# dashpay/agora-blsful

Measured on AMD Instinct MI355X. Metric: BLS12-381 sig verifications/sec (batch), higher is better.
Workload: dtype u32

## Files before the change

### agora-blsful_amd/csrc/h2c.cuh

```cuda
#pragma once
#include "curve.cuh"
#include "tower_split.cuh"

struct sha256_ctx {
  uint32_t h[8];
  uint32_t w[16];
  uint32_t cur;
  uint32_t fill;
  uint32_t total;
};

BLS_CONST uint32_t SHA256_K[64] = {
    0x428a2f98, 0x71374491, 0xb5c0fbcf, 0xe9b5dba5, 0x3956c25b, 0x59f111f1, 0x923f82a4, 0xab1c5ed5, 0xd807aa98, 0x12835b01,
    0x243185be, 0x550c7dc3, 0x72be5d74, 0x80deb1fe, 0x9bdc06a7, 0xc19bf174, 0xe49b69c1, 0xefbe4786, 0x0fc19dc6, 0x240ca1cc,
    0x2de92c6f, 0x4a7484aa, 0x5cb0a9dc, 0x76f988da, 0x983e5152, 0xa831c66d, 0xb00327c8, 0xbf597fc7, 0xc6e00bf3, 0xd5a79147,
    0x06ca6351, 0x14292967, 0x27b70a85, 0x2e1b2138, 0x4d2c6dfc, 0x53380d13, 0x650a7354, 0x766a0abb, 0x81c2c92e, 0x92722c85,
    0xa2bfe8a1, 0xa81a664b, 0xc24b8b70, 0xc76c51a3, 0xd192e819, 0xd6990624, 0xf40e3585, 0x106aa070, 0x19a4c116, 0x1e376c08,
    0x2748774c, 0x34b0bcb5, 0x391c0cb3, 0x4ed8aa4a, 0x5b9cca4f, 0x682e6ff3, 0x748f82ee, 0x78a5636f, 0x84c87814, 0x8cc70208,
    0x90befffa, 0xa4506ceb, 0xbef9a3f7, 0xc67178f2};

BLS_FN uint32_t rotr32(uint32_t x, int n) { return (x >> n) | (x << (32 - n)); }

BLS_FN void sha256_rounds(uint32_t* h, const uint32_t* wsrc) {
  uint32_t w[16];
// ... 125 lines not shown
  uint32_t w[16];
  uint32_t nw;
};
BLS_FN void sha_words_block(sha_words& s) {
#if defined(__HIPCC__)
  u32x8_t hv;
  u32x16_t wv;
#pragma unroll
  for (int i = 0; i < 8; i++) hv[i] = s.h[i];
#pragma unroll
  for (int i = 0; i < 16; i++) wv[i] = s.w[i];
  hv = sha256_compress_v(hv, wv);
#pragma unroll
  for (int i = 0; i < 8; i++) s.h[i] = hv[i];
#else
  sha256_rounds(s.h, s.w);
#endif
}
BLS_FN void sha_words_init(sha_words& s) {
  s.h[0] = 0x6a09e667; s.h[1] = 0xbb67ae85; s.h[2] = 0x3c6ef372; s.h[3] = 0xa54ff53a;
  s.h[4] = 0x510e527f; s.h[5] = 0x9b05688c; s.h[6] = 0x1f83d9ab; s.h[7] = 0x5be0cd19;
#pragma unroll
  for (int i = 0; i < 16; i++) s.w[i] = 0;
  s.nw = 0;
}
BLS_FN void sha_words_feed(sha_words& s, uint32_t word) {
#pragma unroll
  for (int i = 0; i < 15; i++) s.w[i] = s.w[i + 1];
  s.w[15] = word;
  if (++s.nw == 16) {
    sha_words_block(s);
    s.nw = 0;
  }
}
BLS_FN uint32_t xmd_tail_word(uint32_t j, uint32_t nhead, uint32_t head, const uint8_t* dst, uint32_t dst_len) {
  uint32_t word = 0;
#pragma unroll
  for (int k = 0; k < 4; k++) {
    const uint32_t q = j + k;
    uint32_t b;
    if (q < nhead) b = (head >> (8 * (nhead - 1 - q))) & 0xffu;
    else if (q - nhead < dst_len) b = dst[q - nhead];
    else if (q - nhead == dst_len) b = dst_len;
    else if (q - nhead == dst_len + 1) b = 0x80u;
    else b = 0;
    word = (word << 8) | b;
  }
  return word;
}
BLS_FN void xmd_finish(sha_words& s, uint32_t before, uint32_t nhead, uint32_t head, const uint8_t* dst, uint32_t dst_len) {
  const uint32_t need = nhead + dst_len + 2, total = before + nhead + dst_len + 1;
  for (uint32_t j = 0; j < need || s.nw != 14; j += 4) sha_words_feed(s, xmd_tail_word(j, nhead, head, dst, dst_len));
  sha_words_feed(s, total >> 29);
  sha_words_feed(s, total << 3);
}
BLS_FN uint32_t be32_at(const uint8_t* p) { return ((uint32_t)p[0] << 24) | ((uint32_t)p[1] << 16) | ((uint32_t)p[2] << 8) | p[3]; }
template <int NOUT>
BLS_FN void expand_message_xmd_words(uint32_t* out, const uint8_t* pre, uint32_t pre_len, const uint8_t* m, uint32_t m_len,
                                     const uint8_t* dst, uint32_t dst_len) {
  if ((pre_len | m_len) & 3u) {
    uint8_t ub[NOUT];
    expand_message_xmd<NOUT>(ub, pre, pre_len, m, m_len, dst, dst_len);
    for (int i = 0; i < NOUT / 4; i++) out[i] = be32_at(ub + 4 * i);
    return;
  }
  sha_words s;
  sha_words_init(s);
  for (int i = 0; i < 16; i++) sha_words_feed(s, 0);
  for (uint32_t i = 0; i < pre_len; i += 4) sha_words_feed(s, be32_at(pre + i));
  if (((size_t)m & 3u) == 0) {
    for (uint32_t i = 0; i < m_len; i += 4) {
      const uint32_t v = *(const uint32_t*)(m + i);
      sha_words_feed(s, (v >> 24) | ((v >> 8) & 0xff00u) | ((v << 8) & 0xff0000u) | (v << 24));
    }
  } else {
    for (uint32_t i = 0; i < m_len; i += 4) sha_words_feed(s, be32_at(m + i));
  }
  xmd_finish(s, 64 + pre_len + m_len, 3, (uint32_t)NOUT << 8, dst, dst_len);
  uint32_t b0[8], bi[8];
#pragma unroll
  for (int i = 0; i < 8; i++) {
    b0[i] = s.h[i];
    bi[i] = 0;
  }
  const int TW = 24;
  const uint32_t need1 = dst_len + 3;
  const bool cached = need1 <= 4 * TW;
  uint32_t T[TW];
  if (cached) {
#pragma unroll
    for (int k = 0; k < TW; k++) T[k] = xmd_tail_word(4 * k, 1, 0, dst, dst_len);
  }
  for (int blk = 1; blk <= NOUT / 32; blk++) {
    sha_words_init(s);
#pragma unroll
    for (int i = 0; i < 8; i++) sha_words_feed(s, b0[i] ^ bi[i]);
    if (cached) {
#pragma unroll
      for (int k = 0; k < TW; k++)
        if (4u * k < need1 || s.nw != 14) sha_words_feed(s, k == 0 ? T[0] | ((uint32_t)blk << 24) : T[k]);
      while (s.nw != 14) sha_words_feed(s, 0);
      sha_words_feed(s, 0);
      sha_words_feed(s, (34 + dst_len) << 3);
    } else {
      xmd_finish(s, 32, 1, (uint32_t)blk, dst, dst_len);
    }
#pragma unroll
    for (int i = 0; i < 8; i++) {
      bi[i] = s.h[i];
      out[8 * (blk - 1) + i] = bi[i];
    }
  }
}
BLS_FN void fp_from_be64_words(fp& r, const uint32_t* wbe) {
  fp lo, hi, t, k;
  uint32_t w[12];
#pragma unroll
  for (int i = 0; i < 12; i++) w[i] = i < 4 ? wbe[3 - i] : 0;
  fp_set_words(hi, w);
#pragma unroll
  for (int i = 0; i < 12; i++) w[i] = wbe[15 - i];
  fp_set_words(lo, w);
  fp_load(k, FP_R2);
  fp_mul(t, k, lo);
  fp_load(k, FP_R2_384);
  fp_mul(hi, k, hi);
  fp_add(t, t, hi);
  fp_reduce(r, t);
}

BLS_FN void fp_from_be64(fp& r, const uint8_t* b) {
  fp lo, hi, t, k;
  uint32_t w[12];
  for (int i = 0; i < 12; i++) w[i] = 0;
  for (int i = 0; i < 4; i++) {
    const uint8_t* q = b + 4 * (3 - i);
    w[i] = ((uint32_t)q[0] << 24) | ((uint32_t)q[1] << 16) | ((uint32_t)q[2] << 8) | q[3];
  }
  fp_set_words(hi, w);
  for (int i = 0; i < 12; i++) {
    const uint8_t* q = b + 16 + 4 * (11 - i);
    w[i] = ((uint32_t)q[0] << 24) | ((uint32_t)q[1] << 16) | ((uint32_t)q[2] << 8) | q[3];
  }
  fp_set_words(lo, w);
  fp_load(k, FP_R2);
  fp_mul(t, k, lo);
  fp_load(k, FP_R2_384);
  fp_mul(hi, k, hi);
  fp_add(t, t, hi);
  fp_reduce(r, t);
}

template <class F>
BLS_NOINLINE void sswu_g1(F& xn, F& xd, F& y, const F& u) {
  F A, B, Z, tv1, tv2, tv3, tv4, tv5, tv6, x, y1, t;
  fp_load(A, SSWU1_A);
  fp_load(B, SSWU1_B);
  fp_load(Z, SSWU1_Z);
  fp_sqr(tv1, u);
  fp_mul(tv1, Z, tv1);
  fp_sqr(tv2, tv1);
  fp_add(tv2, tv2, tv1);
  fp_one(t);
  fp_add(tv3, tv2, t);
  fp_mul(tv3, B, tv3);
  fp_neg(tv4, tv2);
  fp_cmov(tv4, Z, fp_is_zero(tv2));
  fp_mul(tv4, A, tv4);
  fp_sqr(tv2, tv3);
  fp_sqr(tv6, tv4);
  fp_mul(tv5, A, tv6);
  fp_add(tv2, tv2, tv5);
  fp_mul(tv2, tv2, tv3);
  fp_mul(tv6, tv6, tv4);
  fp_mul(tv5, B, tv6);
  fp_add(tv2, tv2, tv5);
  fp_mul(x, tv1, tv3);
  F s1, s2, s3, y2, c2;
  fp_sqr(s1, tv6);
  fp_mul(s2, tv2, tv6);
  fp_mul(s1, s1, s2);
  fp_pow(y1, s1, EXP_PM3D4, EXP_PM3D4_BITS);
  fp_mul(y1, y1, s2);
  fp_load(c2, SSWU1_C2);
  fp_mul(y2, y1, c2);
  fp_sqr(s3, y1);
  fp_mul(s3, s3, tv6);
  bool is_qr = fp_eq(s3, tv2);
  fp_mul(y, tv1, u);
  fp_mul(y, y, y2);
  fp_cmov(x, tv3, is_qr);
  fp_cmov(y, y1, is_qr);
  F ny;
  fp_neg(ny, y);
  fp_cmov(y, ny, fp_parity(u) != fp_parity(y));
  xn = x;
  xd = tv4;
}

BLS_NOINLINE void iso_map_g1(g1_jac& r, const fp& xn, const fp& xd, const fp& y) {
  fp XN, XD, YN, YD, pw, c, t;
  fp_load(XN, ISO1_XNUM[11]);
  fp_load(XD, ISO1_XDEN[10]);
  fp_load(YN, ISO1_YNUM[15]);
  fp_load(YD, ISO1_YDEN[15]);
  pw = xd;
#pragma unroll
  for (int j = 1; j <= 15; j++) {
    if (j > 1) fp_mul(pw, pw, xd);
    if (j <= 11) {
      fp_mul(XN, XN, xn);
      fp_load(c, ISO1_XNUM[11 - j]);
      fp_mul(t, c, pw);
      fp_add(XN, XN, t);
    }
    if (j <= 10) {
      fp_mul(XD, XD, xn);
      fp_load(c, ISO1_XDEN[10 - j]);
      fp_mul(t, c, pw);
      fp_add(XD, XD, t);
    }
    fp_mul(YN, YN, xn);
    fp_load(c, ISO1_YNUM[15 - j]);
    fp_mul(t, c, pw);
    fp_add(YN, YN, t);
    fp_mul(YD, YD, xn);
    fp_load(c, ISO1_YDEN[15 - j]);
    fp_mul(t, c, pw);
    fp_add(YD, YD, t);
  }
  fp zx, yd2;
  fp_mul(zx, XD, xd);
  fp_mul(r.z, zx, YD);
  fp_sqr(yd2, YD);
  fp_mul(t, XN, zx);
  fp_mul(r.x, t, yd2);
  fp_sqr(t, zx);
  fp_mul(t, t, zx);
  fp_mul(t, t, yd2);
  fp_mul(t, t, YN);
  fp_mul(r.y, t, y);
}

#if defined(__HIPCC__)
__device__ __forceinline__ void fp_lane_swap(fp& r, const fp& a) {
#pragma unroll
  for (int i = 0; i < FP_NL; i++) r.l[i] = dpp_swap(a.l[i]);
}
__device__ __forceinline__ void jac_dbl_pair(g1_jac& p, bool hi) {
  fp s1, s2, s3, in, a, b, o2, o3, D, E, t, x3, y3, z3, c8;
  fp_sel(in, hi, p.y, p.x);
  fp_sqr(s1, in);
  fp_dbl(E, s1);
  fp_add(E, E, s1);
  fp_reduce(E, E);
  fp_sel(in, hi, s1, E);
  fp_sqr(s2, in);
  fp_add(t, p.x, s1);
  fp_sel(a, hi, t, p.y);
  fp_sel(b, hi, t, p.z);
  fp_mul(s3, a, b);
  fp_lane_swap(o2, s2);
  fp_lane_swap(o3, s3);
  fp_sub(t, o3, s1);
  fp_sub(t, t, o2);
  fp_dbl(D, t);
  fp_reduce(D, D);
  fp_dbl(t, D);
  fp_sub(t, s2, t);
  fp_reduce(x3, t);
  fp_sub(t, D, x3);
  fp_mul(t, E, t);
  fp_dbl(c8, o2);
  fp_dbl(c8, c8);
  fp_reduce(c8, c8);
  fp_dbl(c8, c8);
  fp_sub(t, t, c8);
  fp_reduce(y3, t);
  fp_dbl(z3, s3);
  fp_reduce(z3, z3);
  fp_lane_swap(a, x3);
  fp_lane_swap(b, y3);
  fp_lane_swap(t, z3);
  fp_sel(p.x, hi, a, x3);
  fp_sel(p.y, hi, b, y3);
  fp_sel(p.z, hi, t, z3);
}
__device__ __noinline__ void jac_mul_u64_pair(g1_jac& r, const g1_jac& p, uint64_t k, bool hi) {
  g1_jac acc;
  jac_set_inf(acc);
  for (int i = 63; i >= 0; i--) {
    jac_dbl_pair(acc, hi);
    if ((k >> i) & 1) jac_add_body(acc, acc, p);
  }
  r = acc;
}
#endif
BLS_NOINLINE void hash_to_g1(g1_jac& r, const uint8_t* pre, uint32_t pre_len, const uint8_t* m, uint32_t m_len,
                       const uint8_t* dst, uint32_t dst_len, int lane2 = -1, bool no_clear = false) {
  uint32_t ub[32];
  expand_message_xmd_words<128>(ub, pre, pre_len, m, m_len, dst, dst_len);
  fp u0, u1, xn, xd, y;
  g1_jac q0, q1;
#if defined(__HIPCC__)
  if (lane2 >= 0) {
    g1_jac mine, other;
    fp_from_be64_words(u0, ub + 16 * lane2);
    sswu_g1(xn, xd, y, u0);
    iso_map_g1(mine, xn, xd, y);
    fp_lane_swap(other.x, mine.x);
    fp_lane_swap(other.y, mine.y);
    fp_lane_swap(other.z, mine.z);
    q0 = lane2 ? other : mine;
    q1 = lane2 ? mine : other;
  } else
#endif
  {
    (void)lane2;
    fp_from_be64_words(u0, ub);
    fp_from_be64_words(u1, ub + 16);
    sswu_g1(xn, xd, y, u0);
    iso_map_g1(q0, xn, xd, y);
    sswu_g1(xn, xd, y, u1);
    iso_map_g1(q1, xn, xd, y);
  }
  jac_add(q0, q0, q1);
  if (no_clear) {
    r = q0;
    return;
  }
#if defined(__HIPCC__)
  if (lane2 >= 0) jac_mul_u64_pair(q1, q0, BLS_X_ABS, lane2 != 0);
  else
#endif
    jac_mul_u64(q1, q0, BLS_X_ABS);
  jac_add(r, q1, q0);
}

template <class F2>
BLS_NOINLINE void sswu_g2(F2& x, F2& y, const F2& u) {
  typedef decltype(F2::c0) F;
  F2 A, B, Z, tv1, tv2, xn, xd, xd2, xd3, num, w, t, Y;
  fp2_load(A, SSWU2_A);
  fp2_load(B, SSWU2_B);
  fp2_load(Z, SSWU2_Z);
  fp2_sqr(tv1, u);
  fp2_mul(tv1, Z, tv1);
  fp2_sqr(tv2, tv1);
  fp2_add(tv2, tv2, tv1);
  fp2_reduce(tv2, tv2);
  fp2_one(t);
  fp2_add(t, tv2, t);
  fp2_mul(xn, B, t);
  fp2_neg(t, tv2);
  fp2_cmov(t, Z, fp2_is_zero(tv2));
  fp2_mul(xd, A, t);
  fp2_sqr(xd2, xd);
  fp2_mul(xd3, xd2, xd);
  fp2_sqr(num, xn);
  fp2_mul(t, A, xd2);
  fp2_add(num, num, t);
  fp2_mul(num, num, xn);
  fp2_mul(t, B, xd3);
  fp2_add(num, num, t);
  fp2_mul(w, num, xd);
  F nxd, nt, inxd;
  fp_sqr(nxd, xd.c0);
  fp_sqr(nt, xd.c1);
  fp_add(nxd, nxd, nt);
  fp_reduce(nxd, nxd);
  F n, sn, c2, nu, nu3, cz, root;
  fp_sqr(n, w.c0);
  fp_sqr(nt, w.c1);
  fp_add(n, n, nt);
  fp_reduce(n, n);
  fp_pow(sn, n, EXP_PM3D4, EXP_PM3D4_BITS);
  fp_mul(sn, sn, n);
  fp_sqr(c2, sn);
  const bool sq1 = fp_eq(c2, n);
  fp_sqr(nu, u.c0);
  fp_sqr(nt, u.c1);
  fp_add(nu, nu, nt);
  fp_reduce(nu, nu);
  fp_sqr(nu3, nu);
  fp_mul(nu3, nu3, nu);
  fp_load(cz, SSWU2_CZ);
  fp_mul(root, sn, cz);
  fp_mul(root, root, nu3);
  fp_cmov(root, sn, sq1);
  {
    F2 t3, w2, xn2;
    fp2_sqr(t3, tv1);
    fp2_mul(t3, t3, tv1);
    fp2_mul(w2, w, t3);
    fp2_mul(xn2, tv1, xn);
    fp2_cmov(w2, w, sq1);
    fp2_cmov(xn2, xn, sq1);
    w = w2;
    xn = xn2;
  }
  if (fp_is_zero(w.c1)) {
    fp2_sqrt_inv(Y, w, &nxd, &inxd);
  } else {
    F h, tt, s, d, prod, pi;
    fp_load(h, FP_HALF);
    fp_add(tt, w.c0, root);
    fp_mul(tt, tt, h);
    fp_pow(s, tt, EXP_PM3D4, EXP_PM3D4_BITS);
    fp_mul(s, s, tt);
    fp_sqr(c2, s);
    const bool direct = fp_eq(c2, tt);
    fp_dbl(d, s);
    fp_reduce(d, d);
    fp_mul(prod, d, nxd);
    fp_inv(pi, prod);
    fp_mul(inxd, pi, d);
    fp_mul(d, pi, nxd);
    fp_mul(d, w.c1, d);
    Y.c0 = s;
    Y.c1 = d;
    F2 alt;
    alt.c0 = d;
    alt.c1 = s;
    fp2_cmov(Y, alt, !direct);
  }
  F2 xdi;
  fp2_conj(xdi, xd);
  fp2_mul_fp(xdi, xdi, inxd);
  fp2_mul(x, xn, xdi);
  fp2_sqr(t, xdi);
  fp2_mul(y, Y, t);
  if (fp2_sgn0(u) != fp2_sgn0(y)) fp2_neg(y, y);
}
template <class F2>
BLS_FN void iso2_poly(F2& r, const uint32_t (*k)[2 * FP_NL], int deg, const F2& x) {
  F2 acc, c;
  fp2_load(acc, k[deg]);
  for (int i = deg - 1; i >= 0; i--) {
    fp2_mul(acc, acc, x);
    fp2_load(c, k[i]);
    fp2_add(acc, acc, c);
  }
  r = acc;
}
BLS_NOINLINE void iso_map_g2(g2_jac& r, const fp2& x, const fp2& y) {
  fp2 XN, XD, YN, YD, t, yd2;
  iso2_poly(XN, ISO2_XNUM, 3, x);
  iso2_poly(XD, ISO2_XDEN, 2, x);
  iso2_poly(YN, ISO2_YNUM, 3, x);
  iso2_poly(YD, ISO2_YDEN, 3, x);
  fp2_mul(r.z, XD, YD);
  fp2_sqr(yd2, YD);
  fp2_mul(t, XN, XD);
  fp2_mul(r.x, t, yd2);
  fp2_sqr(t, XD);
  fp2_mul(t, t, XD);
  fp2_mul(t, t, yd2);
  fp2_mul(t, t, YN);
  fp2_mul(r.y, t, y);
}
template <class F2>
BLS_FN void iso_map_g2_hom(F2& X, F2& Y, F2& Z, const F2& x, const F2& y) {
  F2 XN, XD, YN, YD, t;
  iso2_poly(XN, ISO2_XNUM, 3, x);
  iso2_poly(XD, ISO2_XDEN, 2, x);
  iso2_poly(YN, ISO2_YNUM, 3, x);
  iso2_poly(YD, ISO2_YDEN, 3, x);
  fp2_mul(X, XN, YD);
  fp2_mul(t, YN, XD);
  fp2_mul(Y, t, y);
  fp2_mul(Z, XD, YD);
}
BLS_NOINLINE void hash_to_g2(g2_jac& r, const uint8_t* pre, uint32_t pre_len, const uint8_t* m, uint32_t m_len,
                       const uint8_t* dst, uint32_t dst_len, int lane2 = -1, bool no_clear = false) {
  uint32_t ub[64];
  expand_message_xmd_words<256>(ub, pre, pre_len, m, m_len, dst, dst_len);
  fp2 u0, u1, x, y;
  g2_jac q0, q1;
#if defined(__HIPCC__)
  if (lane2 >= 0) {
    g2_jac mine, other;
    fp_from_be64_words(u0.c0, ub + 32 * lane2);
    fp_from_be64_words(u0.c1, ub + 32 * lane2 + 16);
    sswu_g2(x, y, u0);
    iso_map_g2(mine, x, y);
    fp_lane_swap(other.x.c0, mine.x.c0);
    fp_lane_swap(other.x.c1, mine.x.c1);
    fp_lane_swap(other.y.c0, mine.y.c0);
    fp_lane_swap(other.y.c1, mine.y.c1);
    fp_lane_swap(other.z.c0, mine.z.c0);
// ... 40 lines not shown
```

### agora-blsful_amd/csrc/kernels.cuh

```cuda
#pragma once
#ifndef BLS_SPLIT_WAVES
#define BLS_SPLIT_WAVES 2
#endif
#include "verify.cuh"

#define BLS_BLOCK 64
#define W1 FP_NL
#define W2 (2 * FP_NL)
#define WS_PAIRS_WORDS (6 * W2)
#define WS_PAIR1_WORDS (3 * W2)
#define WS_F_WORDS (6 * W2)
#define LINE5_WORDS (5 * FP_NL)
#define LINE3_WORDS_H (3 * FP_NL)
#define FX_STORE_WORDS (10 * 6 * FP_NL)
#define MILLER1_GROUP 3

struct dst_arg {
  uint8_t b[256];
  uint32_t len;
};

__device__ __forceinline__ void ws_ld_fp(fp& r, const uint32_t* ws, size_t stride, size_t i, int w0) {
#pragma unroll
  for (int k = 0; k < FP_NL; k++) r.l[k] = (int32_t)ws[(size_t)(w0 + k) * stride + i];
// ... 196 lines not shown
}

template <int SG>
__global__ void k_prepare(size_t n, const uint8_t* pks, const uint8_t* sigs, int fmt, int aug, const uint8_t* msgs,
                          const uint64_t* offs, int single_msg, dst_arg dst, uint32_t* pairs, int32_t* status, int pre_status, int two_lanes);
__global__ void k_miller2s(size_t n, const uint32_t* pairs, const int32_t* status, uint32_t* fws, int fixed_g2);
__global__ void k_lines2s(size_t n, size_t first, size_t count, const uint32_t* pairs, const int32_t* status, uint32_t* lines, uint32_t* lines3, size_t lanes, int fixed_g2, int pass);
__global__ void k_millerf2s(size_t n, size_t first, size_t count, const int32_t* status, const uint32_t* lines, size_t lanes, uint32_t* fws);
__global__ void k_finalexp2s(size_t n, size_t first, size_t count, const uint32_t* fws, uint32_t* vp, size_t lanes, int32_t* status);
__global__ void k_finalexp_seg(int seg, size_t n, size_t first, size_t count, const uint32_t* fws, uint32_t* vp, size_t lanes, int32_t* status);
__global__ void k_cyc_run4(size_t count, uint32_t* vp, size_t lanes, const int32_t* status, size_t first);
__global__ void k_linesp(size_t mm, size_t half, size_t stride, const uint32_t* pairs, const int32_t* bad, uint32_t* lines, uint32_t* lines3, size_t lanes, size_t first_v, size_t count_v, int pass);
__global__ void k_linesp4(size_t cnt, size_t stride, const uint32_t* pairs, const int32_t* bad, uint32_t* lines3, size_t lanes);
__global__ void k_lines_fixed(size_t stride, const uint32_t* pairs, const int32_t* bad, uint32_t* lines3, size_t lanes, int fixed_g2);
__global__ void k_millerfp(size_t count_v, size_t q, int group, const uint32_t* lines, size_t lanes, uint32_t* fws, size_t stride, size_t out0);
__global__ void k_millerfp3(size_t count, size_t q, int group, const int32_t* bad, const uint32_t* lines3, size_t lanes, uint32_t* fws, size_t stride, size_t out0);
__global__ void k_line_quad(size_t count, size_t q, const int32_t* bad, const uint32_t* lines3, size_t lanes, uint32_t* fout, size_t sout, size_t rout, size_t oout);
__global__ void k_f12_fold4(size_t qin, size_t qout, int fan, const uint32_t* fin, size_t sin, size_t rin, uint32_t* fout, size_t sout, size_t rout, size_t oout);
__global__ void k_finalexps(size_t n, const uint32_t* fws, int32_t* status);
__global__ void k_miller1s(size_t n, size_t stride, const uint32_t* pairs, const int32_t* skip, uint32_t* fws);
__global__ void k_finalexp_ones(const uint32_t* fws, size_t stride, int32_t* verdict);
__global__ void k_pairing_coop(size_t n, const uint32_t* pairs, int32_t* status, int fixed_g2);
__global__ void k_finalexp_coop(const uint32_t* fws, size_t stride, int32_t* verdict);
template <int SG>
__global__ void k_prepare_agg(size_t n, const uint8_t* pks, const uint8_t* sig, int fmt, int aug, const uint8_t* msgs,
                              const uint64_t* offs, dst_arg dst, uint32_t* pairs, int32_t* bad, int two_lanes, int has_sig);
__global__ void k_pairs_to_affine(size_t n, const uint8_t* g1s, const uint8_t* g2s, int fmt, uint32_t* pairs, int32_t* skip);
__global__ void k_pairs2_to_affine(size_t n, const uint8_t* g1a, const uint8_t* g2a, const uint8_t* g1b, const uint8_t* g2b, int fmt,
                                   uint32_t* pairs, int32_t* status);
__global__ void k_status_to_flag(size_t n, int32_t* status);
template <int SG>
__global__ void k_prepare_hashed(size_t n, const uint8_t* pks, const uint8_t* sigs, const uint8_t* hashes, uint32_t* pairs, int32_t* status, int fmt);
template <int SG>
__global__ void k_prepare_proof(size_t n, const uint8_t* commitments, const uint8_t* proofs, const uint8_t* pks, const uint8_t* ys,
                                int fmt, const uint8_t* msgs, const uint64_t* offs, dst_arg dst, uint32_t* pairs, int32_t* status);
__global__ void k_f12_fold(size_t m, size_t half, uint32_t* fws, size_t stride);
#define GROUPED_ITEMS 8
template <int SG>
__global__ void k_prepare_grouped(size_t n, const uint8_t* pks, const uint8_t* sigs, int fmt, int aug, const uint8_t* msgs, const uint64_t* offs,
                                  dst_arg dst, uint64_t seed, size_t ng, uint32_t* pairs, int32_t* skip, uint8_t* scaled_sigs, int32_t* status);
__global__ void k_group_sigsum(size_t ng, size_t n, const uint8_t* scaled_sigs, uint32_t* pairs, int32_t* skip);
__global__ void k_f12_mul3(size_t ng, const uint32_t* fin, size_t stride_in, uint32_t* fout);
__global__ void k_f12_import(size_t n, const uint8_t* src, uint32_t* fws, size_t stride);
__global__ void k_f12_export(const uint32_t* fws, size_t stride, uint8_t* dst);
__global__ void k_hash_to_g1(size_t n, const uint8_t* msgs, const uint64_t* offs, dst_arg dst, uint8_t* out, int two_lanes);
__global__ void k_hash_to_g2(size_t n, const uint8_t* msgs, const uint64_t* offs, dst_arg dst, uint8_t* out, int two_lanes);
template <int G, int WITH_SCALARS>
__global__ void k_accumulate(size_t n, const uint8_t* pts, int fmt, const uint8_t* scalars, const uint32_t* perm,
                             uint8_t* partials, size_t T);
__global__ void k_accumulate_g2s(size_t n, const uint8_t* pts, int fmt, uint8_t* partials, size_t T);
template <int G>
__global__ void k_point_fold(size_t m, size_t half, uint8_t* partials);
__global__ void k_point_fold_g2s(size_t m, size_t half, uint8_t* partials);
template <int G>
__global__ void k_compress(size_t n, const uint8_t* pts, int fmt, int legacy, uint8_t* out);
template <int SG>
__global__ void k_sign(size_t n, const uint8_t* sks, int aug, const uint8_t* msgs, const uint64_t* offs, dst_arg dst,
                       uint8_t* out_pks, uint8_t* out_sigs);
__global__ void k_msm_count(size_t n, const uint8_t* scalars, int c, int W, int clast, uint32_t* cnt);
__global__ void k_msm_fill(size_t n, const uint8_t* scalars, int c, int W, int clast, const uint32_t* off, uint32_t* cursor, uint32_t* idx);
template <int G>
__global__ void k_msm_bucket(size_t nb, const uint8_t* pts, int fmt, const uint32_t* perm, const uint32_t* cnt, const uint32_t* off,
                             const uint32_t* idx, uint8_t* sums);
template <int G>
__global__ void k_msm_chunk(int c, int W, int clast, int CH, const uint8_t* sums, uint8_t* partials);
__global__ void k_msm_chunk_g2s(int c, int W, int clast, int CH, const uint8_t* sums, uint8_t* partials);
__global__ void k_msm_chunk_g1p(int c, int W, int clast, int CH, const uint8_t* sums, uint8_t* partials);
__global__ void k_msm_chunk_g2q(int c, int W, int clast, int CH, const uint8_t* sums, uint8_t* partials);
__global__ void k_msm_bucket_g2s(size_t nb, const uint8_t* pts, int fmt, const uint32_t* perm, const uint32_t* cnt, const uint32_t* off,
                                 const uint32_t* idx, uint8_t* sums);
template <int G>
__global__ void k_normalize(uint8_t* pt);
#define MSM2_E(G) ((G) == 1 ? 2 : 4)
#define MSM2_AFF_WORDS(G) ((G) == 1 ? 2 * FP_NL : 4 * FP_NL)
template <int G>
__global__ void k_msm2_prep(size_t n, const uint8_t* pts, int fmt, const uint32_t* perm, uint32_t* affws, uint8_t* inf);
template <int G>
__global__ void k_msm2_tables(size_t n, const uint32_t* affws, const uint8_t* inf, int W, uint32_t* tab, uint32_t* jt);
template <int G>
__global__ void k_msm2_count(size_t n, const uint8_t* scalars, const uint8_t* inf, int W, uint32_t* cnt, uint64_t* subs);
template <int G>
__global__ void k_msm2_fill(size_t n, const uint64_t* subs, const uint8_t* inf, int W, const uint32_t* off, uint32_t* cursor, uint32_t* idx);
__global__ void k_msm2_merge_g1(size_t nb, int Q, uint8_t* sums);
__global__ void k_msm2_merge_g2s(size_t nb, int Q, uint8_t* sums);
__global__ void k_msm2_bucket_g1(size_t nb, int Q, const uint32_t* affws, const uint32_t* cnt, const uint32_t* off, const uint32_t* idx, uint8_t* sums, int tabW);
__global__ void k_msm2_bucket_g2s(size_t nb, int Q, const uint32_t* affws, const uint32_t* cnt, const uint32_t* off, const uint32_t* idx, uint8_t* sums, int tabW);
__global__ void k_msm2_chunk_g1p(int W, int CH, int stride, const uint8_t* sums, uint8_t* partials, int weighted);
__global__ void k_msm2_chunk_g2q(int W, int CH, int stride, const uint8_t* sums, uint8_t* partials, int weighted);
template <int G>
__global__ void k_decompress(size_t n, const uint8_t* bytes, int legacy, uint8_t* out, int32_t* status, int keep);

#include "util_kernels.cuh"
__global__ void k_wide_mul_test(size_t n, const uint8_t* a, const uint8_t* b, uint8_t* out, int reps);
#include "wide_rows.cuh"
#define WIDE_BLOCK 256
#define WIDE_ENGINE_BLOCK (16 * WIDE_TABLE_ROWS)
#define WIDE_EASY_WORDS (12 * 16)
__global__ void k_pairing_coop_easy(size_t n, const uint32_t* pairs, const int32_t* status, int fixed_g2, uint32_t* easy);
__global__ void k_finalexp_wide(size_t n, const uint32_t* easy, int32_t* status);
__global__ void k_finalexp_wide_ws(const uint32_t* fws, size_t stride, int32_t* verdict);
__global__ void k_f12_tree_wide(size_t m, const uint32_t* fin, size_t sin, uint32_t* fout, size_t sout);
__global__ void k_f12_tree_seg(size_t qin, const uint32_t* fin, size_t sin, size_t rin, uint32_t* fout, size_t sout, size_t rout);
__global__ void k_f12_horner_wide(const uint32_t* fin, size_t sin, uint32_t* fout, size_t sout);
__global__ void k_wide_prog_test(const uint32_t* prog, int len, int reps, const uint8_t* fin, uint8_t* tout);
bool wide_prog_is_fp12(const uint32_t* prog, size_t len);
__global__ void k_pairing_wide(size_t n, const uint32_t* pairs, int32_t* status, int fixed_g2);
__global__ void k_hash_to_g1_wide(size_t n, const uint8_t* msgs, const uint64_t* offs, int single_msg, dst_arg dst, uint8_t* out, uint32_t* rec);
__global__ void k_hash_to_g1_engine(size_t n, const uint8_t* msgs, const uint64_t* offs, int single_msg, dst_arg dst, uint8_t* out, uint32_t* rec);
#define WREC_P0 0
#define WREC_P1 3
#define WREC_Q0 6
#define WREC_F1 12
#define WREC_L 24
#define WREC_Q1 (24 + 6 * 68)
#define WREC_F2 (WREC_Q1 + 6)
#define WREC_F2_SLOTS 2
#define WREC_VALUES (WREC_F2 + 12 * WREC_F2_SLOTS)
#define WREC_WORDS (16 * WREC_VALUES)
template <int SG>
__global__ void k_prepare_keys(size_t n, const uint8_t* pks, const uint8_t* sigs, const uint8_t* hashes, int fmt, int parts, uint32_t* rec, int32_t* status);
__global__ void k_pairing_pre(size_t n, uint32_t* rec, const int32_t* status, int first_part, int second_part);
__global__ void k_pairing_post(size_t n, const uint32_t* rec, int32_t* status);
#define WSTREAM_FLAGS 32
#define WSTREAM_MAX_ITEMS 64
#define WPOST2_MAX_ITEMS 128
#define WSTREAM_SPIN_LIMIT (1u << 21)
#define BLS_ERR_STREAM_TIMEOUT (-2)
__global__ void k_pairing_stream(size_t n, uint32_t* rec, int32_t* status, uint32_t* flags, uint32_t epoch);
__global__ void k_pairing_post2(size_t n, uint32_t* rec, int32_t* status, uint32_t* flags, uint32_t epoch);
template <int G>
__global__ void k_point_tree_wide(size_t m, const uint8_t* in, uint8_t* out);
__global__ void k_g2_clear_wide(size_t n, uint8_t* pts);
__global__ void k_hash_to_g2_engine(size_t n, const uint8_t* msgs, const uint64_t* offs, int single_msg, dst_arg dst, uint8_t* out, uint32_t* rec);
__global__ void k_hash_to_g2_maps(size_t n, const uint8_t* msgs, const uint64_t* offs, int single_msg, dst_arg dst, uint32_t* pts);
__global__ void k_g2_hash_tail_wide(size_t n, const uint32_t* pts, uint8_t* out, uint32_t* rec);

#if defined(BLS_TU_PREPARE1) || defined(BLS_TU_PREPARE2)
template <int SG>
__global__ void __launch_bounds__(BLS_BLOCK, 2) k_prepare(size_t n, const uint8_t* pks, const uint8_t* sigs, int fmt, int aug,
                                                     const uint8_t* msgs, const uint64_t* offs, int single_msg, dst_arg dst,
                                                     uint32_t* pairs, int32_t* status, int pre_status, int two_lanes) {
  const size_t gid = (size_t)blockIdx.x * blockDim.x + threadIdx.x;
  const bool tl = SG == 2 || (two_lanes & 1) != 0;
  const size_t i = tl ? gid >> 1 : gid;
  const int lane2 = tl ? (int)(gid & 1) : -1;
  if (i >= n) return;
  if (pre_status && status[i] != BLS_OK) return;
  size_t mi = single_msg ? 0 : i;
  const uint8_t* m = msgs + offs[mi];
  uint32_t mlen = (uint32_t)(offs[mi + 1] - offs[mi]);
  g1_aff P[2];
  g2_aff Q[2];
  int st;
  if (SG == 1 && !aug) {
    fp zs;
    fp2 zp;
    load_g1_z(zs, sigs, i, fmt);
    load_g2_z(zp, pks, i, fmt);
    if (fp_is_zero(zs)) {
      st = BLS_ERR_SIG_IDENTITY;
    } else if (fp2_is_zero(zp)) {
      st = BLS_ERR_PK_IDENTITY;
    } else {
      const bool no_clear = (two_lanes & 2) != 0;
      g1_jac h;
      hash_to_g1(h, nullptr, 0, m, mlen, dst.b, dst.len, lane2, no_clear);
      g2_jac pk;
      g1_jac sig;
      load_g2_pt(pk, pks, i, fmt);
      load_g1_pt(sig, sigs, i, fmt);
      prepare_g1impl_tail(P, Q, pk, sig, h);
      if (no_clear) g2_negc_gen(Q[1]);
      else g2_neg_gen(Q[1]);
      st = BLS_OK;
    }
  } else if (SG == 1) {
    g2_jac pk;
    g1_jac sig;
    load_g2_pt(pk, pks, i, fmt);
    load_g1_pt(sig, sigs, i, fmt);
    st = prepare_g1impl(P, Q, pk, sig, aug, m, mlen, dst.b, dst.len, lane2, (two_lanes & 2) != 0);
  } else {
    g1_jac pk;
    g2_jac sig;
    load_g1_pt(pk, pks, i, fmt);
    load_g2_pt(sig, sigs, i, fmt);
    st = prepare_g2impl(P, Q, pk, sig, aug, m, mlen, dst.b, dst.len, lane2);
  }
  if (lane2 > 0) return;
  status[i] = st;
  if (st != BLS_OK) return;
  ws_st_pair(pairs, n, i, 0, P[0], Q[0]);
  ws_st_pair(pairs, n, i, 1, P[1], Q[1]);
}
__device__ __forceinline__ void sha256_u64(sha256_ctx& c, uint64_t x) {
  for (int k = 7; k >= 0; k--) sha256_byte(c, (uint8_t)(x >> (8 * k)));
}
struct u128_pair { uint64_t hi, lo; };
__device__ __noinline__ u128_pair grouped_scalar(uint64_t seed, size_t n, size_t i, const uint8_t* pk, uint32_t pk_len, const uint8_t* sig, uint32_t sig_len,
                                              const uint8_t* m, uint32_t mlen) {
  static_assert(GROUPED_ITEMS == 8 && BLS_BLOCK % GROUPED_ITEMS == 0, "a group is an aligned octet of lanes");
  uint8_t d[32];
  sha256_ctx c;
  if (i < n) {
    const char tag[] = "blsgpu-grouped-v3";
    sha256_init(c);
    sha256_update(c, (const uint8_t*)tag, sizeof tag - 1);
    sha256_u64(c, seed);
    sha256_u64(c, (uint64_t)n);
    sha256_u64(c, (uint64_t)i);
    sha256_update(c, pk, pk_len);
    sha256_update(c, sig, sig_len);
    sha256_u64(c, mlen);
    sha256_update(c, m, mlen);
    sha256_final(c, d);
  } else {
    for (int k = 0; k < 32; k++) d[k] = 0;
  }
  uint32_t w[8];
  for (int k = 0; k < 8; k++) w[k] = ((uint32_t)d[4 * k] << 24) | ((uint32_t)d[4 * k + 1] << 16) | ((uint32_t)d[4 * k + 2] << 8) | d[4 * k + 3];
  sha256_init(c);
  for (int j = 0; j < GROUPED_ITEMS; j++)
    for (int k = 0; k < 8; k++) {
      const uint32_t x = (uint32_t)__shfl((int)w[k], j, GROUPED_ITEMS);
      sha256_byte(c, (uint8_t)(x >> 24));
      sha256_byte(c, (uint8_t)(x >> 16));
      sha256_byte(c, (uint8_t)(x >> 8));
      sha256_byte(c, (uint8_t)x);
    }
  sha256_final(c, d);
  sha256_init(c);
  sha256_update(c, d, 32);
  sha256_u64(c, (uint64_t)i);
  sha256_final(c, d);
  u128_pair r{0, 0};
  for (int k = 0; k < 8; k++) r.hi = (r.hi << 8) | d[k];
  for (int k = 8; k < 16; k++) r.lo = (r.lo << 8) | d[k];
  if (!(r.hi | r.lo)) r.lo = 1;
  return r;
}
template <int SG>
__global__ void __launch_bounds__(BLS_BLOCK, 2) k_prepare_grouped(size_t n, const uint8_t* pks, const uint8_t* sigs, int fmt, int aug, const uint8_t* msgs,
                                                             const uint64_t* offs, dst_arg dst, uint64_t seed, size_t ng, uint32_t* pairs, int32_t* skip,
                                                             uint8_t* scaled_sigs, int32_t* status) {
  static_assert(SG == 1, "grouped verification is built for Bls12381G1Impl");
  const size_t i = (size_t)blockIdx.x * blockDim.x + threadIdx.x;
  const bool live = i < n;
  const size_t ii = live ? i : 0;
  const uint8_t* m = msgs + offs[ii];
  const uint32_t mlen = (uint32_t)(offs[ii + 1] - offs[ii]);
  const uint32_t pk_len = fmt == 0 ? 288 : 192, sig_len = fmt == 0 ? 144 : 96;
  const u128_pair r = grouped_scalar(seed, n, i, pks + ii * pk_len, pk_len, sigs + ii * sig_len, sig_len, m, mlen);
  if (!live) return;
  const size_t slot = i / GROUPED_ITEMS + (i % GROUPED_ITEMS) * ng, stride = (GROUPED_ITEMS + 1) * ng;
  g1_aff P[2];
  g2_aff Q[2];
  g2_jac pk;
  g1_jac sig, a, b;
  load_g2_pt(pk, pks, i, fmt);
  load_g1_pt(sig, sigs, i, fmt);
  const int st = prepare_g1impl(P, Q, pk, sig, aug, m, mlen, dst.b, dst.len, -1, true);
  status[i] = st;
  if (st != BLS_OK) {
    jac_set_inf(b);
    store_g1_pt(scaled_sigs, i, b);
    return;
  }
  jac_from_aff(a, P[0]);
  jac_mul_u128(a, a, r.hi, r.lo);
  jac_from_aff(b, P[1]);
  jac_mul_u128(b, b, r.hi, r.lo);
  g1_aff A;
  jac_to_aff(A, a);
  ws_st_pair(pairs, stride, slot, 0, A, Q[0]);
  skip[slot] = A.inf ? 1 : 0;
  store_g1_pt(scaled_sigs, i, b);
}
#if defined(BLS_TU_PREPARE1)
template __global__ void k_prepare_grouped<1>(size_t, const uint8_t*, const uint8_t*, int, int, const uint8_t*, const uint64_t*, dst_arg, uint64_t, size_t,
                                              uint32_t*, int32_t*, uint8_t*, int32_t*);
#endif
#if defined(BLS_TU_PREPARE1)
template __global__ void k_prepare<1>(size_t, const uint8_t*, const uint8_t*, int, int, const uint8_t*, const uint64_t*, int, dst_arg, uint32_t*, int32_t*, int, int);
#else
template __global__ void k_prepare<2>(size_t, const uint8_t*, const uint8_t*, int, int, const uint8_t*, const uint64_t*, int, dst_arg, uint32_t*, int32_t*, int, int);
#endif
#endif



#if defined(BLS_TU_AGG1) || defined(BLS_TU_AGG2) || defined(BLS_TU_AGG_BATCH)
template <int SG>
__device__ __forceinline__ void prepare_agg_item(bool is_sig, const uint8_t* pts, size_t pt_i, int fmt, int aug, const uint8_t* m, uint32_t mlen,
                                                 const dst_arg& dst, uint32_t* pairs, size_t stride, size_t slot, int32_t* bad, int two_lanes, int lane2) {
  g1_aff P;
  g2_aff Q;
  if (is_sig) {
    if (SG == 1) {
      g1_jac s;
      load_g1_pt(s, pts, pt_i, fmt);
      const bool inf = jac_is_inf(s);
      if (lane2 <= 0) bad[slot] = inf ? 1 : 0;
      if (inf) return;
      jac_to_aff(P, s);
      if (two_lanes & 2) g2_negc_gen(Q);
      else g2_neg_gen(Q);
    } else {
      g2_jac s;
      load_g2_pt(s, pts, pt_i, fmt);
      const bool inf = jac_is_inf(s);
      if (lane2 <= 0) bad[slot] = inf ? 1 : 0;
      if (inf) return;
      jac_to_aff(Q, s);
      g1_neg_gen(P);
    }
    if (lane2 <= 0) ws_st_pair(pairs, stride, slot, 0, P, Q);
    return;
  }
  if (SG == 1) {
    g2_jac pk;
    load_g2_pt(pk, pts, pt_i, fmt);
    const bool inf = jac_is_inf(pk);
    if (lane2 <= 0) bad[slot] = inf ? 1 : 0;
    if (inf) return;
    uint8_t pre[96];
    g1_jac h;
    if (aug) {
      jac_to_aff(Q, pk);
      g2_compress(pre, Q, false);
      hash_to_g1(h, pre, 96, m, mlen, dst.b, dst.len, lane2, (two_lanes & 2) != 0);
      jac_to_aff(P, h);
    } else {
      hash_to_g1(h, pre, 0, m, mlen, dst.b, dst.len, lane2, (two_lanes & 2) != 0);
      if (jac_is_inf(h)) {
// ... 3329 lines not shown
```

### agora-blsful_amd/csrc/verify.cuh

```cuda
#pragma once
#include "h2c.cuh"
#include "pairing.cuh"

#define BLS_OK 0
#define BLS_ERR_INVALID_SIGNATURE 1
#define BLS_ERR_SIG_IDENTITY 2
#define BLS_ERR_PK_IDENTITY 3
#define BLS_ERR_DUPLICATE_MESSAGE 4
#define BLS_ERR_INVALID_COEFFICIENT 5
#define BLS_ERR_BAD_LENGTH 6
#define BLS_ERR_BAD_ENCODING 7
#define BLS_ERR_LEGACY_FORMAT 8
#define BLS_ERR_COMMITMENT_IDENTITY 9
#define BLS_ERR_PROOF_IDENTITY 10
#define BLS_ERR_ZERO_CHALLENGE 11

BLS_FN void fp_inv3(fp& a, fp& b, fp& c) {
  fp ab, abc, t;
  fp_mul(ab, a, b);
  fp_mul(abc, ab, c);
  fp_inv(abc, abc);
  fp_mul(t, abc, ab);
  fp_mul(abc, abc, c);
  c = t;
  fp_mul(t, abc, b);
  fp_mul(b, abc, a);
  a = t;
}
BLS_FN void fp_inv2(fp& a, fp& b) {
  fp ab, t;
  fp_mul(ab, a, b);
  fp_inv(ab, ab);
  fp_mul(t, ab, b);
  fp_mul(b, ab, a);
  a = t;
}
BLS_FN void g1_apply_zinv(g1_aff& r, const g1_jac& p, const fp& zi) {
  fp zi2;
  fp_sqr(zi2, zi);
  fp_mul(r.x, p.x, zi2);
  fp_mul(zi2, zi2, zi);
  fp_mul(r.y, p.y, zi2);
  r.inf = false;
}
BLS_FN void g2_apply_ninv(g2_aff& r, const g2_jac& p, const fp& ni) {
  fp2 zi, zi2;
  fp_mul(zi.c0, p.z.c0, ni);
  fp_mul(zi.c1, p.z.c1, ni);
  fp_neg(zi.c1, zi.c1);
  fp2_sqr(zi2, zi);
  fp2_mul(r.x, p.x, zi2);
  fp2_mul(zi2, zi2, zi);
  fp2_mul(r.y, p.y, zi2);
  r.inf = false;
}
BLS_FN void fp2_norm_sq(fp& n, const fp2& a) {
  fp t;
  fp_sqr(n, a.c0);
  fp_sqr(t, a.c1);
  fp_add(n, n, t);
}

BLS_FN void g1g2_to_aff(g1_aff& a1, g2_aff& a2, const g1_jac& p1, const g2_jac& p2) {
  fp z1 = p1.z, n2;
  fp2_norm_sq(n2, p2.z);
  fp_inv2(z1, n2);
  g1_apply_zinv(a1, p1, z1);
  g2_apply_ninv(a2, p2, n2);
}

BLS_FN void g1_neg_gen(g1_aff& r) {
  fp_load(r.x, G1_GEN_X);
  fp y;
  fp_load(y, G1_GEN_Y);
  fp_neg(r.y, y);
  r.inf = false;
}
BLS_FN void g2_negc_gen(g2_aff& r) {
  fp2_load(r.x, G2_NEGC_X);
  fp2_load(r.y, G2_NEGC_Y);
  r.inf = false;
}
BLS_FN void g2_neg_gen(g2_aff& r) {
  fp2_load(r.x, G2_GEN_X);
  fp2 y;
  fp2_load(y, G2_GEN_Y);
  fp2_neg(r.y, y);
  r.inf = false;
}

BLS_FN void prepare_g1impl_tail(g1_aff* P, g2_aff* Q, const g2_jac& pk, const g1_jac& sig, const g1_jac& h) {
  if (jac_is_inf(h)) {
    g1g2_to_aff(P[1], Q[0], sig, pk);
    jac_to_aff(P[0], h);
  } else {
    fp zs = sig.z, zh = h.z, n;
    fp2_norm_sq(n, pk.z);
    fp_inv3(zs, zh, n);
    g1_apply_zinv(P[1], sig, zs);
    g1_apply_zinv(P[0], h, zh);
    g2_apply_ninv(Q[0], pk, n);
  }
}
BLS_FN int prepare_g1impl(g1_aff* P, g2_aff* Q, const g2_jac& pk, const g1_jac& sig, int mode, const uint8_t* msg,
                          uint32_t msg_len, const uint8_t* dst, uint32_t dst_len, int lane2 = -1, bool no_clear = false) {
  if (jac_is_inf(sig)) return BLS_ERR_SIG_IDENTITY;
  if (jac_is_inf(pk)) return BLS_ERR_PK_IDENTITY;
  g1_jac h;
  if (mode) {
    g1g2_to_aff(P[1], Q[0], sig, pk);
    uint8_t pre[96];
    g2_compress(pre, Q[0], false);
    if (mode == 1) hash_to_g1(h, pre, 96, msg, msg_len, dst, dst_len, lane2, no_clear);
    else hash_to_g1(h, nullptr, 0, pre, 96, dst, dst_len, lane2, no_clear);
    jac_to_aff(P[0], h);
  } else {
    hash_to_g1(h, nullptr, 0, msg, msg_len, dst, dst_len, lane2, no_clear);
    prepare_g1impl_tail(P, Q, pk, sig, h);
  }
  if (no_clear) g2_negc_gen(Q[1]);
  else g2_neg_gen(Q[1]);
  return BLS_OK;
}

BLS_FN int prepare_g2impl(g1_aff* P, g2_aff* Q, const g1_jac& pk, const g2_jac& sig, int mode, const uint8_t* msg,
                          uint32_t msg_len, const uint8_t* dst, uint32_t dst_len, int lane2 = -1) {
  if (jac_is_inf(sig)) return BLS_ERR_SIG_IDENTITY;
  if (jac_is_inf(pk)) return BLS_ERR_PK_IDENTITY;
  g2_jac h;
  if (mode) {
    g1g2_to_aff(P[0], Q[1], pk, sig);
    uint8_t pre[48];
    g1_compress(pre, P[0], false);
    if (mode == 1) hash_to_g2(h, pre, 48, msg, msg_len, dst, dst_len, lane2);
    else hash_to_g2(h, nullptr, 0, pre, 48, dst, dst_len, lane2);
    jac_to_aff(Q[0], h);
  } else {
    hash_to_g2(h, nullptr, 0, msg, msg_len, dst, dst_len, lane2);
    if (jac_is_inf(h)) {
      g1g2_to_aff(P[0], Q[1], pk, sig);
      jac_to_aff(Q[0], h);
    } else {
      fp zp = pk.z, ns, nh;
      fp2_norm_sq(ns, sig.z);
      fp2_norm_sq(nh, h.z);
      fp_inv3(zp, ns, nh);
      g1_apply_zinv(P[0], pk, zp);
      g2_apply_ninv(Q[1], sig, ns);
      g2_apply_ninv(Q[0], h, nh);
    }
  }
  g1_neg_gen(P[1]);
  return BLS_OK;
}

template <class F2>
BLS_FN int pairing_verdict(const fp12_t<F2>& f) {
  return final_exp_is_one(f) ? BLS_OK : BLS_ERR_INVALID_SIGNATURE;
}
```

Measured before the change: 3.388 million.

## Pass G1 hash-to-curve intermediates through LDS between noinline stages

Restructures G1 hash-to-curve in the prepare kernel into separate noinline stages (map, add, cofactor multiply, to-affine) that exchange points through a per-thread shared-memory column instead of registers or the stack. The aim is to cut register pressure and scratch spills across call boundaries in the large prepare kernel. The cost is extra LDS traffic, more shared memory per block (which may limit occupancy), and extra call overhead.

```diff
diff --git a/agora-blsful_amd/csrc/h2c.cuh b/agora-blsful_amd/csrc/h2c.cuh
--- a/agora-blsful_amd/csrc/h2c.cuh
+++ b/agora-blsful_amd/csrc/h2c.cuh
@@ -301,7 +301,7 @@
 }
 
 template <class F>
-BLS_NOINLINE void sswu_g1(F& xn, F& xd, F& y, const F& u) {
+BLS_FN void sswu_g1_body(F& xn, F& xd, F& y, const F& u) {
   F A, B, Z, tv1, tv2, tv3, tv4, tv5, tv6, x, y1, t;
   fp_load(A, SSWU1_A);
   fp_load(B, SSWU1_B);
@@ -346,8 +346,12 @@
   xn = x;
   xd = tv4;
 }
-
-BLS_NOINLINE void iso_map_g1(g1_jac& r, const fp& xn, const fp& xd, const fp& y) {
+template <class F>
+BLS_NOINLINE void sswu_g1(F& xn, F& xd, F& y, const F& u) {
+  sswu_g1_body(xn, xd, y, u);
+}
+
+BLS_FN void iso_map_g1_body(g1_jac& r, const fp& xn, const fp& xd, const fp& y) {
   fp XN, XD, YN, YD, pw, c, t;
   fp_load(XN, ISO1_XNUM[11]);
   fp_load(XD, ISO1_XDEN[10]);
@@ -390,6 +394,7 @@
   fp_mul(t, t, YN);
   fp_mul(r.y, t, y);
 }
+BLS_NOINLINE void iso_map_g1(g1_jac& r, const fp& xn, const fp& xd, const fp& y) { iso_map_g1_body(r, xn, xd, y); }
 
 #if defined(__HIPCC__)
 __device__ __forceinline__ void fp_lane_swap(fp& r, const fp& a) {
@@ -435,7 +440,7 @@
   fp_sel(p.y, hi, b, y3);
   fp_sel(p.z, hi, t, z3);
 }
-__device__ __noinline__ void jac_mul_u64_pair(g1_jac& r, const g1_jac& p, uint64_t k, bool hi) {
+__device__ __forceinline__ void jac_mul_u64_pair_body(g1_jac& r, const g1_jac& p, uint64_t k, bool hi) {
   g1_jac acc;
   jac_set_inf(acc);
   for (int i = 63; i >= 0; i--) {
@@ -444,6 +449,7 @@
   }
   r = acc;
 }
+__device__ __noinline__ void jac_mul_u64_pair(g1_jac& r, const g1_jac& p, uint64_t k, bool hi) { jac_mul_u64_pair_body(r, p, k, hi); }
 #endif
 BLS_NOINLINE void hash_to_g1(g1_jac& r, const uint8_t* pre, uint32_t pre_len, const uint8_t* m, uint32_t m_len,
                        const uint8_t* dst, uint32_t dst_len, int lane2 = -1, bool no_clear = false) {
@@ -485,6 +491,105 @@
     jac_mul_u64(q1, q0, BLS_X_ABS);
   jac_add(r, q1, q0);
 }
+
+#if defined(__HIPCC__) && (defined(BLS_TU_PREPARE1) || defined(BLS_TU_PREPARE2))
+#define PW_WORDS (2 * 3 * (FP_NL - 1))
+#define PW_P 0
+#define PW_Q (3 * (FP_NL - 1))
+__device__ __forceinline__ void pw_ld_g1(g1_jac& p, const lds_u32* sh, int w0) {
+  sh_ld_fp(p.x, sh, w0);
+  sh_ld_fp(p.y, sh, w0 + (FP_NL - 1));
+  sh_ld_fp(p.z, sh, w0 + 2 * (FP_NL - 1));
+}
+__device__ __forceinline__ void pw_st_g1(lds_u32* sh, int w0, const g1_jac& p) {
+  sh_st_fp(sh, w0, p.x);
+  sh_st_fp(sh, w0 + (FP_NL - 1), p.y);
+  sh_st_fp(sh, w0 + 2 * (FP_NL - 1), p.z);
+}
+static __device__ __noinline__ void pw_map_g1(lds_u32* sh, int dst) {
+  fp u, xn, xd, y;
+  g1_jac r;
+  shu_ld_fp(u, sh, dst);
+  sswu_g1_body(xn, xd, y, u);
+  iso_map_g1_body(r, xn, xd, y);
+  pw_st_g1(sh, dst, r);
+}
+static __device__ __noinline__ void pw_add_g1(lds_u32* sh, int dst, int a, int b) {
+  g1_jac p, q, r;
+  pw_ld_g1(p, sh, a);
+  pw_ld_g1(q, sh, b);
+  jac_add_body(r, p, q);
+  pw_st_g1(sh, dst, r);
+}
+static __device__ __noinline__ void pw_mul_u64_g1(lds_u32* sh, uint64_t k, int lane2) {
+  g1_jac p, r;
+  pw_ld_g1(p, sh, PW_P);
+  if (lane2 >= 0) {
+    jac_mul_u64_pair_body(r, p, k, lane2 != 0);
+  } else {
+    g1_jac acc;
+    jac_set_inf(acc);
+    for (int i = 63; i >= 0; i--) {
+      jac_dbl_body(acc, acc);
+      if ((k >> i) & 1) jac_add_body(acc, acc, p);
+    }
+    r = acc;
+  }
+  pw_st_g1(sh, PW_Q, r);
+}
+__device__ __forceinline__ void pw_pair_exchange_g1(lds_u32* sh, bool hi) {
+#pragma unroll
+  for (int k = 0; k < 3 * (FP_NL - 1); k++) {
+    const int32_t own = (int32_t)sh[(PW_P + k) * BLS_SH_STRIDE], other = dpp_swap(own);
+    sh[(PW_P + k) * BLS_SH_STRIDE] = (uint32_t)(hi ? other : own);
+    sh[(PW_Q + k) * BLS_SH_STRIDE] = (uint32_t)(hi ? own : other);
+  }
+}
+static __device__ __noinline__ int pw_to_aff_g1(lds_u32* sh) {
+  g1_jac p;
+  g1_aff a;
+  pw_ld_g1(p, sh, PW_P);
+  if (jac_is_inf(p)) {
+    a.inf = true;
+    fe_zero(a.x);
+    fe_zero(a.y);
+  } else {
+    fp zi, zi2;
+    fe_inv(zi, p.z);
+    fe_sqr(zi2, zi);
+    fe_mul(a.x, p.x, zi2);
+    fe_mul(zi2, zi2, zi);
+    fe_mul(a.y, p.y, zi2);
+    a.inf = false;
+  }
+  sh_st_fp(sh, PW_P, a.x);
+  sh_st_fp(sh, PW_P + (FP_NL - 1), a.y);
+  return a.inf ? 1 : 0;
+}
+__device__ __noinline__ void hash_to_g1_pw(lds_u32* sh, const uint8_t* pre, uint32_t pre_len, const uint8_t* m, uint32_t m_len,
+                                           const uint8_t* dst, uint32_t dst_len, int lane2, bool no_clear) {
+  uint32_t ub[32];
+  expand_message_xmd_words<128>(ub, pre, pre_len, m, m_len, dst, dst_len);
+  fp u;
+  if (lane2 >= 0) {
+    fp_from_be64_words(u, ub + 16 * lane2);
+    shu_st_fp(sh, PW_P, u);
+    pw_map_g1(sh, PW_P);
+    pw_pair_exchange_g1(sh, lane2 != 0);
+  } else {
+    fp_from_be64_words(u, ub);
+    shu_st_fp(sh, PW_P, u);
+    pw_map_g1(sh, PW_P);
+    fp_from_be64_words(u, ub + 16);
+    shu_st_fp(sh, PW_Q, u);
+    pw_map_g1(sh, PW_Q);
+  }
+  pw_add_g1(sh, PW_P, PW_P, PW_Q);
+  if (no_clear) return;
+  pw_mul_u64_g1(sh, BLS_X_ABS, lane2);
+  pw_add_g1(sh, PW_P, PW_Q, PW_P);
+}
+#endif
 
 template <class F2>
 BLS_NOINLINE void sswu_g2(F2& x, F2& y, const F2& u) {
diff --git a/agora-blsful_amd/csrc/kernels.cuh b/agora-blsful_amd/csrc/kernels.cuh
--- a/agora-blsful_amd/csrc/kernels.cuh
+++ b/agora-blsful_amd/csrc/kernels.cuh
@@ -372,6 +372,11 @@
   g1_aff P[2];
   g2_aff Q[2];
   int st;
+  lds_u32* sh = nullptr;
+  if constexpr (SG == 1) {
+    __shared__ uint32_t pw[PW_WORDS * BLS_BLOCK];
+    sh = lds_column(pw);
+  }
   if (SG == 1 && !aug) {
     fp zs;
     fp2 zp;
@@ -383,13 +388,12 @@
       st = BLS_ERR_PK_IDENTITY;
     } else {
       const bool no_clear = (two_lanes & 2) != 0;
-      g1_jac h;
-      hash_to_g1(h, nullptr, 0, m, mlen, dst.b, dst.len, lane2, no_clear);
+      hash_to_g1_pw(sh, nullptr, 0, m, mlen, dst.b, dst.len, lane2, no_clear);
       g2_jac pk;
       g1_jac sig;
       load_g2_pt(pk, pks, i, fmt);
       load_g1_pt(sig, sigs, i, fmt);
-      prepare_g1impl_tail(P, Q, pk, sig, h);
+      prepare_g1impl_tail_pw(P, Q, pk, sig, sh);
       if (no_clear) g2_negc_gen(Q[1]);
       else g2_neg_gen(Q[1]);
       st = BLS_OK;
@@ -399,7 +403,7 @@
     g1_jac sig;
     load_g2_pt(pk, pks, i, fmt);
     load_g1_pt(sig, sigs, i, fmt);
-    st = prepare_g1impl(P, Q, pk, sig, aug, m, mlen, dst.b, dst.len, lane2, (two_lanes & 2) != 0);
+    st = prepare_g1impl_pw(P, Q, pk, sig, aug, m, mlen, dst.b, dst.len, lane2, (two_lanes & 2) != 0, sh);
   } else {
     g1_jac pk;
     g2_jac sig;
diff --git a/agora-blsful_amd/csrc/verify.cuh b/agora-blsful_amd/csrc/verify.cuh
--- a/agora-blsful_amd/csrc/verify.cuh
+++ b/agora-blsful_amd/csrc/verify.cuh
@@ -122,6 +122,47 @@
   else g2_neg_gen(Q[1]);
   return BLS_OK;
 }
+
+#if defined(__HIPCC__) && (defined(BLS_TU_PREPARE1) || defined(BLS_TU_PREPARE2))
+BLS_FN void prepare_g1impl_tail_pw(g1_aff* P, g2_aff* Q, const g2_jac& pk, const g1_jac& sig, lds_u32* sh) {
+  g1_jac h;
+  pw_ld_g1(h, sh, PW_P);
+  if (jac_is_inf(h)) {
+    g1g2_to_aff(P[1], Q[0], sig, pk);
+    P[0].inf = pw_to_aff_g1(sh) != 0;
+    sh_ld_fp(P[0].x, sh, PW_P);
+    sh_ld_fp(P[0].y, sh, PW_P + (FP_NL - 1));
+  } else {
+    fp zs = sig.z, zh = h.z, n;
+    fp2_norm_sq(n, pk.z);
+    fp_inv3(zs, zh, n);
+    g1_apply_zinv(P[1], sig, zs);
+    g1_apply_zinv(P[0], h, zh);
+    g2_apply_ninv(Q[0], pk, n);
+  }
+}
+BLS_FN int prepare_g1impl_pw(g1_aff* P, g2_aff* Q, const g2_jac& pk, const g1_jac& sig, int mode, const uint8_t* msg, uint32_t msg_len,
+                             const uint8_t* dst, uint32_t dst_len, int lane2, bool no_clear, lds_u32* sh) {
+  if (jac_is_inf(sig)) return BLS_ERR_SIG_IDENTITY;
+  if (jac_is_inf(pk)) return BLS_ERR_PK_IDENTITY;
+  if (mode) {
+    g1g2_to_aff(P[1], Q[0], sig, pk);
+    uint8_t pre[96];
+    g2_compress(pre, Q[0], false);
+    if (mode == 1) hash_to_g1_pw(sh, pre, 96, msg, msg_len, dst, dst_len, lane2, no_clear);
+    else hash_to_g1_pw(sh, nullptr, 0, pre, 96, dst, dst_len, lane2, no_clear);
+    P[0].inf = pw_to_aff_g1(sh) != 0;
+    sh_ld_fp(P[0].x, sh, PW_P);
+    sh_ld_fp(P[0].y, sh, PW_P + (FP_NL - 1));
+  } else {
+    hash_to_g1_pw(sh, nullptr, 0, msg, msg_len, dst, dst_len, lane2, no_clear);
+    prepare_g1impl_tail_pw(P, Q, pk, sig, sh);
+  }
+  if (no_clear) g2_negc_gen(Q[1]);
+  else g2_neg_gen(Q[1]);
+  return BLS_OK;
+}
+#endif
 
 BLS_FN int prepare_g2impl(g1_aff* P, g2_aff* Q, const g1_jac& pk, const g2_jac& sig, int mode, const uint8_t* msg,
                           uint32_t msg_len, const uint8_t* dst, uint32_t dst_len, int lane2 = -1) {
```

Measured after the change: 3.361 million. No clear change (-0.8%).
